# Huangying-Zhan/DF-VO

Measured on NVIDIA H100. Metric: VO frames/sec on 376x1241 pairs, higher is better.
Workload: dtype bf16 tensor-core convs (fp32 accumulate) + fp32 flow/selection + fp64 pose solvers

## Files before the change

df-vo_b200/csrc/conv_chain.cu:

```cuda
#include "tc_ptx.cuh"

#ifndef DFVO_HOSTSIM
#include <cuda.h>
#include <stdio.h>
#include <stdlib.h>
#include <string.h>

#include <vector>

namespace dfvo {

#define CHAIN_MAXL 12
#define CHAIN_THREADS 384
#define CHAIN_TH 16

struct ChainL {
  int N, H, W, tiles_x, tiles_y, n_blocks, ntiles;
  int nsrc, srcC[3];
  int kh, kw, dy0, dx0, HW, HH;
  int block_n;
  int Cout, Cout_pad, act, out_f32, zero_pad_to;
  const float* bias;
  void* out; long long oN, oH, oW;
  const void* res; long long rN, rH, rW;
// ... 97 lines not shown
      const int ntaps = p.kh * p.kw;
      const uint32_t b_bytes = (uint32_t)p.block_n * 128u;
      for (int tile = blockIdx.x; tile < p.ntiles; tile += gridDim.x) {
        const int nb = tile / (p.tiles_x * p.tiles_y * p.N);
        int kofs = 0;
        for (int s = 0; s < p.nsrc; ++s) {
          for (int c0 = 0; c0 < p.srcC[s]; c0 += 64) {
            for (int tap = 0; tap < ntaps; ++tap) {
              mbar_wait(rb.empty(), rb.ph ^ 1u);
              if (elect_one()) {
                mbar_expect_tx(rb.full(), b_bytes);
                tma_load_3d(rb.slot(), &P.tmB[l], rb.full(), kofs + c0, nb * p.block_n, tap);
              }
              __syncwarp();
              rb.next();
            }
          }
          kofs += p.srcC[s];
        }
      }
    }
  } else if (warp >= 4) {
    const int ct = threadIdx.x - 128, wg = ct >> 7, wq = (ct >> 5) & 3;
    const bool leader = (ct & 127) == 0;
    for (int l = 0; l < P.nlayers; ++l) {
      const ChainL& p = P.L[l];
      asm volatile("bar.sync 1, 256;" ::: "memory");
      for (int i = ct; i < p.Cout_pad; i += 256) bias_s[i] = p.bias ? p.bias[i] : 0.f;
      asm volatile("bar.sync 1, 256;" ::: "memory");
      if (l > 0 && p.res != nullptr) {
        if (lane == 0 && !chain_wait(P.bar + (l - 1), gridDim.x)) *P.err = 1u;
        __syncwarp();
      }
      TcEpi ep; ep.Cout = p.Cout; ep.zero_pad_to = p.zero_pad_to; ep.act = p.act; ep.out_f32 = p.out_f32; ep.round_tf32 = 0; ep.out = p.out; ep.res = p.res;
      switch (p.block_n) {
        case 16: chain_layer<S, 16>(p, ra, rb, ep, bias_s, wg, wq, lane, leader); break;
        case 32: chain_layer<S, 32>(p, ra, rb, ep, bias_s, wg, wq, lane, leader); break;
        case 64: chain_layer<S, 64>(p, ra, rb, ep, bias_s, wg, wq, lane, leader); break;
        case 128: if (S <= 2) chain_layer<S, (S <= 2 ? 128 : 16)>(p, ra, rb, ep, bias_s, wg, wq, lane, leader); break;
        default: if (S == 1) chain_layer<S, (S == 1 ? 256 : 16)>(p, ra, rb, ep, bias_s, wg, wq, lane, leader); break;
      }
      if (l + 1 < P.nlayers) {
        asm volatile("fence.proxy.async;" ::: "memory");
        __threadfence();
        asm volatile("bar.sync 1, 256;" ::: "memory");
        if (ct == 0) chain_arrive(P.bar + l);
      }
    }
  }
}

static int chain_env(const char* name, int dflt) {
  const char* v = getenv(name);
  return v ? atoi(v) : dflt;
}

static bool chain_rect(const ConvTc& c, int* kh, int* kw, int* dy0, int* dx0) {
  int ymin = 127, ymax = -128, xmin = 127, xmax = -128;
  for (int t = 0; t < c.ntaps; ++t) {
    if (c.dy[t] < ymin) ymin = c.dy[t];
    if (c.dy[t] > ymax) ymax = c.dy[t];
    if (c.dx[t] < xmin) xmin = c.dx[t];
    if (c.dx[t] > xmax) xmax = c.dx[t];
  }
  const int h = ymax - ymin + 1, w = xmax - xmin + 1;
  if (h * w != c.ntaps) return false;
  for (int t = 0; t < c.ntaps; ++t)
// ... 198 lines not shown
```

df-vo_b200/csrc/conv_halo.cu:

```cuda
#include "tc_ptx.cuh"

#ifndef DFVO_HOSTSIM
#include <cuda.h>
#include <stdio.h>
#include <stdlib.h>
#include <string.h>

namespace dfvo {

struct ConvHaloK {
  int N, H, W, tiles_x, tiles_y, n_blocks, ntiles;
  int nsrc, srcC[3];
  int kh, kw, dy0, dx0;
  int HW, HH;
  int a_stages, b_stages, a_stage_bytes;
  int Cout, Cout_pad, act, out_f32, zero_pad_to;
  int chunk;
  int esize, round_tf32;
  const float* bias;
  void* out; long long oN, oH, oW;
  const void* res; long long rN, rH, rW;
};

#define HALO_THREADS 384
#define HALO_TH 16

template <int S, int BN, int TF32, int MINB>
__global__ void __launch_bounds__(HALO_THREADS, MINB)
k_conv_halo(const __grid_constant__ CUtensorMap tmA0, const __grid_constant__ CUtensorMap tmA1,
            const __grid_constant__ CUtensorMap tmA2, const __grid_constant__ CUtensorMap tmB,
            const __grid_constant__ ConvHaloK p) {
  using namespace tc;
  extern __shared__ uint8_t smem_raw[];
  const uint32_t raw = smem_u32(smem_raw);
  const uint32_t base = (raw + 1023u) & ~1023u;
  uint8_t* base_ptr = smem_raw + (base - raw);
  const uint32_t b_stage_bytes = (uint32_t)BN * 128u;
  const uint32_t a_base = base;
  const uint32_t b_base = base + (uint32_t)p.a_stages * (uint32_t)p.a_stage_bytes;
  const uint32_t bar_base = b_base + (uint32_t)p.b_stages * b_stage_bytes;
  TcRing ra{a_base, (uint32_t)p.a_stage_bytes, bar_base, bar_base + 8u * (uint32_t)p.a_stages, p.a_stages, 0, 0u};
  TcRing rb{b_base, b_stage_bytes, bar_base + 16u * (uint32_t)p.a_stages, bar_base + 16u * (uint32_t)p.a_stages + 8u * (uint32_t)p.b_stages,
            p.b_stages, 0, 0u};
  float* bias_s = reinterpret_cast<float*>(base_ptr + (bar_base - base) + 16u * (uint32_t)(p.a_stages + p.b_stages));

  const int warp = threadIdx.x >> 5, lane = threadIdx.x & 31;

  pdl_trigger();

  if (warp == 0 && lane == 0) {
    prefetch_tmap(&tmA0); prefetch_tmap(&tmB);
// ... 20 lines not shown
          if (elect_one()) {
            mbar_expect_tx(ra.full(), a_bytes);
            tma_load_4d(ra.slot(), tm, ra.full(), c0, x0, y0, n);
          }
          __syncwarp();
          ra.next();
        }
      }
    }
  } else if (warp == 1) {
    for (int tile = blockIdx.x; tile < p.ntiles; tile += gridDim.x) {
      const int nb = tile / (p.tiles_x * p.tiles_y * p.N);
      int kofs = 0;
      for (int s = 0; s < p.nsrc; ++s) {
        for (int c0 = 0; c0 < p.srcC[s]; c0 += p.chunk) {
          for (int tap = 0; tap < ntaps; ++tap) {
            mbar_wait(rb.empty(), rb.ph ^ 1u);
            if (elect_one()) {
              mbar_expect_tx(rb.full(), b_stage_bytes);
              tma_load_3d(rb.slot(), &tmB, rb.full(), kofs + c0, nb * BN, tap);
            }
            __syncwarp();
            rb.next();
          }
        }
        kofs += p.srcC[s];
      }
    }
  } else if (warp >= 4) {
    const int ct = threadIdx.x - 128, wg = ct >> 7;
    for (int i = ct; i < p.Cout_pad; i += 256) bias_s[i] = p.bias ? p.bias[i] : 0.f;
    asm volatile("bar.sync 1, 256;" ::: "memory");
    TcEpi ep; ep.Cout = p.Cout; ep.zero_pad_to = p.zero_pad_to; ep.act = p.act; ep.out_f32 = p.out_f32; ep.round_tf32 = p.round_tf32; ep.out = p.out; ep.res = p.res;
    float acc[S][BN / 2];
    for (int tile = blockIdx.x; tile < p.ntiles; tile += gridDim.x) {
      halo_tile_mma<S, BN, TF32>(acc, ra, rb, p.nsrc, p.srcC, p.chunk, p.esize, p.kh, p.kw, p.HW, wg, (ct & 127) == 0);
      int t = tile;
      const int tx = t % p.tiles_x; t /= p.tiles_x;
      const int ty = t % p.tiles_y; t /= p.tiles_y;
      const int n = t % p.N; const int nb = t / p.N;
      halo_tile_store<S, BN>(acc, ep, bias_s, nb * BN, n, tx * 8 * S, ty * HALO_TH, p.W, p.H, p.oN, p.oH, p.oW, p.rN, p.rH, p.rW, wg,
                             (ct >> 5) & 3, lane);
    }
  }
}

static int env_int(const char* name, int dflt) {
  const char* v = getenv(name);
  return v ? atoi(v) : dflt;
}

static bool rect_taps(const ConvTc& c, int* kh, int* kw, int* dy0, int* dx0) {
  int ymin = 127, ymax = -128, xmin = 127, xmax = -128;
  for (int t = 0; t < c.ntaps; ++t) {
    if (c.dy[t] < ymin) ymin = c.dy[t];
    if (c.dy[t] > ymax) ymax = c.dy[t];
    if (c.dx[t] < xmin) xmin = c.dx[t];
    if (c.dx[t] > xmax) xmax = c.dx[t];
  }
  const int h = ymax - ymin + 1, w = xmax - xmin + 1;
  if (h * w != c.ntaps) return false;
  for (int t = 0; t < c.ntaps; ++t)
    if (c.dy[t] != ymin + t / w || c.dx[t] != xmin + t % w) return false;
  *kh = h; *kw = w; *dy0 = ymin; *dx0 = xmin;
  return true;
}

struct HaloCfg { int S, block_n, ctas, a_stages, b_stages, a_stage_bytes; size_t smem; double cost; };

static bool halo_fit(int S, int bn, int ctas, int kh, int kw, int Cout_pad, HaloCfg* out) {
  const int HW = 8 * S + kw - 1, HH = HALO_TH + kh - 1;
  if (HW > 256 || HH > 256) return false;
  const int a_stage = (HW * HH * 128 + 1023) & ~1023;
  const int b_stage = bn * 128;
  const size_t fixed = 1024 + 8 * 64 + (size_t)Cout_pad * 4;
// ... 78 lines not shown
#undef DFVO_HALO_CASE
  DFVO_REQUIRE(false, DFVO_EINVAL, "conv_halo: no kernel for S %d block_n %d with %d CTAs per SM", S, bn, ctas);
}

int conv_halo(const ConvTc& c, cudaStream_t s) {
  DFVO_REQUIRE(c.nsrc >= 1 && c.nsrc <= 3 && c.ntaps >= 1 && c.ntaps <= 49, DFVO_EINVAL, "conv_halo: nsrc/ntaps");
  DFVO_REQUIRE(c.Cout_pad % 16 == 0 && c.Cout_pad >= 16, DFVO_EINVAL, "conv_halo: Cout_pad %d must be a multiple of 16", c.Cout_pad);
  ConvHaloK k;
  memset(&k, 0, sizeof(k));
  DFVO_REQUIRE(rect_taps(c, &k.kh, &k.kw, &k.dy0, &k.dx0), DFVO_EINVAL, "conv_halo: taps are not a rectangle");
  HaloCfg h;
  DFVO_REQUIRE(halo_choose(c, k.kh, k.kw, &h), DFVO_EINVAL, "conv_halo: no tile configuration fits");
  const int S = h.S, bn = h.block_n;
  k.N = c.N; k.H = c.H; k.W = c.W;
  k.tiles_x = cdiv(c.W, 8 * S); k.tiles_y = cdiv(c.H, HALO_TH);
  k.n_blocks = c.Cout_pad / bn;
  k.ntiles = k.tiles_x * k.tiles_y * c.N * k.n_blocks;
  k.HW = 8 * S + k.kw - 1; k.HH = HALO_TH + k.kh - 1;
  k.a_stages = h.a_stages; k.b_stages = h.b_stages; k.a_stage_bytes = h.a_stage_bytes;
  k.nsrc = c.nsrc;
  const int es = c.esize == 4 ? 4 : 2;
  k.esize = es; k.chunk = 128 / es; k.round_tf32 = c.round_out_tf32;
  int ktot = 0;
  for (int i = 0; i < c.nsrc; ++i) {
    DFVO_REQUIRE(c.src[i].C % 16 == 0 && c.src[i].C > 0, DFVO_EINVAL, "conv_halo: source %d channels %d not a multiple of 16", i, c.src[i].C);
    DFVO_REQUIRE(((uintptr_t)c.src[i].p & 15) == 0 && (c.src[i].sW * es) % 16 == 0 && (c.src[i].sH * es) % 16 == 0 && (c.src[i].sN * es) % 16 == 0,
                 DFVO_EINVAL, "conv_halo: source %d not 16-byte aligned/strided", i);
    k.srcC[i] = c.src[i].C; ktot += c.src[i].C;
  }
  k.Cout = c.Cout; k.Cout_pad = c.Cout_pad; k.act = c.act; k.out_f32 = c.out_f32;
  k.zero_pad_to = c.zero_pad_to > c.Cout ? c.zero_pad_to : c.Cout;
  k.bias = c.bias; k.out = c.out; k.oN = c.oN; k.oH = c.oH; k.oW = c.oW;
  k.res = c.residual; k.rN = c.rN; k.rH = c.rH; k.rW = c.rW;

  CUtensorMap tmA[3], tmB;
  for (int i = 0; i < 3; ++i) {
    const ConvTcSource& src = c.src[i < c.nsrc ? i : 0];
    const int inW = c.inW > 0 ? c.inW : c.W, inH = c.inH > 0 ? c.inH : c.H;
    unsigned long long dims[4] = {(unsigned long long)src.C, (unsigned long long)inW, (unsigned long long)inH, (unsigned long long)c.N};
    unsigned long long str[3] = {(unsigned long long)src.sW * es, (unsigned long long)src.sH * es, (unsigned long long)src.sN * es};
    unsigned box[4] = {(unsigned)k.chunk, (unsigned)k.HW, (unsigned)k.HH, 1};
    int rc = tc_encode_map(&tmA[i], src.p, 4, dims, str, box, es);
    if (rc) return rc;
  }
  {
    unsigned long long dims[3] = {(unsigned long long)ktot, (unsigned long long)c.Cout_pad, (unsigned long long)c.ntaps};
    unsigned long long str[2] = {(unsigned long long)ktot * es, (unsigned long long)ktot * es * (unsigned long long)c.Cout_pad};
    unsigned box[3] = {(unsigned)k.chunk, (unsigned)bn, 1};
    int rc = tc_encode_map(&tmB, c.w, 3, dims, str, box, es);
    if (rc) return rc;
  }
  const int slots = h.ctas * tc_num_sms();
  const int grid = k.ntiles < slots ? k.ntiles : slots;
  ++g_launch_count;
  TcProf pr;
  const bool prof = tc_prof_begin(s, &pr);
  const int rc = es == 4 ? launch_halo_t<1>(S, bn, h.ctas, tmA, tmB, k, grid, h.smem, s) : launch_halo_t<0>(S, bn, h.ctas, tmA, tmB, k, grid, h.smem, s);
  if (rc) return rc;
  if (prof) {
    char d[256];
    snprintf(d, sizeof(d), "halo%s N%d %dx%d k%dx%d src[%d,%d,%d] cout%d/%d bn%d S%d stages%d/%d grid%d tiles%d ctas%d gflop %.3f", es == 4 ? "-tf32" : "", c.N, c.H, c.W,
             k.kh, k.kw, c.src[0].C, c.nsrc > 1 ? c.src[1].C : 0, c.nsrc > 2 ? c.src[2].C : 0, c.Cout, c.Cout_pad, bn,
             S, k.a_stages, k.b_stages, grid, k.ntiles, h.ctas, c.flops * 1e-9);
    tc_prof_end(s, pr, c.flops, d);
  }
  DFVO_CHECK_LAUNCH();
  return DFVO_OK;
}

}
#endif
```

df-vo_b200/csrc/conv_tc.cu:

```cuda
#include "tc_ptx.cuh"

#ifndef DFVO_HOSTSIM
#include <cuda.h>
#endif
#include <stdio.h>
#include <stdlib.h>
#include <string.h>

#include <string>
#include <utility>
#include <vector>

namespace dfvo {

void conv_tc_tile_shape(int H, int W, int* tw, int* th) {
  long long best = -1;
  int bw = 128, bh = 1;
  for (int w = 128; w >= 1; w >>= 1) {
    int h = 128 / w;
    long long area = (long long)cdiv(W, w) * w * (long long)cdiv(H, h) * h;
    if (best < 0 || area < best) { best = area; bw = w; bh = h; }
  }
  *tw = bw; *th = bh;
}

struct ConvTcK {
  int N, H, W, tw, th, tiles_x, tiles_y, n_blocks, ntiles;
  int nsrc, srcC[3];
  int ntaps;
  int8_t dy[49], dx[49];
  int8_t py[49], px[49];
  int stride, src_pitch;
  int block_n, stages;
  int Cout, Cout_pad, act, out_f32, zero_pad_to;
  int chunk, esize, round_tf32;
  const float* bias;
  void* out; long long oN, oH, oW;
  const void* res; long long rN, rH, rW;
};

#ifndef DFVO_HOSTSIM
#define TC_THREADS 384
#define TC_A_BYTES 16384

template <int BN, int TF32, int NKS>
__device__ __forceinline__ void tc_stage_mma(float (&acc)[1][BN / 2], uint32_t at, uint32_t bt, uint32_t fresh) {
  using namespace tc;
  wgmma_fence();
  halo_tap_mma<1, BN, TF32, NKS>(acc, at, bt, 1024u, fresh);
  wgmma_commit();
  wgmma_wait<1>();
}

template <int BN, int TF32>
__global__ void __launch_bounds__(TC_THREADS, 1)
k_conv_tc(const __grid_constant__ CUtensorMap tmA0, const __grid_constant__ CUtensorMap tmA1,
          const __grid_constant__ CUtensorMap tmA2, const __grid_constant__ CUtensorMap tmB,
          const __grid_constant__ ConvTcK p) {
  using namespace tc;
  extern __shared__ uint8_t smem_raw[];
  const uint32_t raw = smem_u32(smem_raw);
  const uint32_t base = (raw + 1023u) & ~1023u;
  uint8_t* base_ptr = smem_raw + (base - raw);
  const uint32_t stage_bytes = TC_A_BYTES + (uint32_t)BN * 128u;
  const uint32_t bar_base = base + (uint32_t)p.stages * stage_bytes;
  auto full_bar = [&](int s) { return bar_base + 8u * (uint32_t)s; };
  auto empty_bar = [&](int s) { return bar_base + 8u * (uint32_t)(p.stages + s); };
  float* bias_s = reinterpret_cast<float*>(base_ptr + (size_t)p.stages * stage_bytes + 8u * (2 * p.stages) + 64);
// ... 16 lines not shown
      int t = tile;
      const int tx = t % p.tiles_x; t /= p.tiles_x;
      const int ty = t % p.tiles_y; t /= p.tiles_y;
      const int n = t % p.N; const int nb = t / p.N;
      const int x0 = tx * p.tw, y0 = ty * p.th;
      for (int tap = 0; tap < p.ntaps; ++tap) {
        int kofs = 0;
        for (int s = 0; s < p.nsrc; ++s) {
          const CUtensorMap* tm = s == 0 ? &tmA0 : (s == 1 ? &tmA1 : &tmA2);
          for (int c0 = 0; c0 < p.srcC[s]; c0 += p.chunk) {
            mbar_wait(empty_bar(stage), phase ^ 1u);
            if (elect_one()) {
              const uint32_t sa = base + (uint32_t)stage * stage_bytes;
              mbar_expect_tx(full_bar(stage), stage_bytes);
              if (p.stride == 2)
                tma_load_5d(sa, tm, full_bar(stage), c0 + p.px[tap] * p.src_pitch, x0 + p.dx[tap], p.py[tap], y0 + p.dy[tap], n);
              else
                tma_load_4d(sa, tm, full_bar(stage), c0, x0 + p.dx[tap], y0 + p.dy[tap], n);
              tma_load_3d(sa + TC_A_BYTES, &tmB, full_bar(stage), kofs + c0, nb * BN, tap);
            }
            __syncwarp();
            if (++stage == p.stages) { stage = 0; phase ^= 1u; }
          }
          kofs += p.srcC[s];
        }
      }
    }
  } else if (warp >= 4) {
    const int ct = threadIdx.x - 128, wg = ct >> 7, wq = (ct >> 5) & 3;
    const bool leader = (ct & 127) == 0;
    for (int i = ct; i < p.Cout_pad; i += 256) bias_s[i] = p.bias ? p.bias[i] : 0.f;
    asm volatile("bar.sync 1, 256;" ::: "memory");
    TcEpi ep; ep.Cout = p.Cout; ep.zero_pad_to = p.zero_pad_to; ep.act = p.act; ep.out_f32 = p.out_f32; ep.round_tf32 = p.round_tf32; ep.out = p.out; ep.res = p.res;
    int stage = 0; uint32_t phase = 0;
    float acc[BN / 2];
    for (int tile = blockIdx.x; tile < p.ntiles; tile += gridDim.x) {
      uint32_t fresh = 0;
      int pend = -1;
      for (int tap = 0; tap < p.ntaps; ++tap) {
        for (int s = 0; s < p.nsrc; ++s) {
          for (int c0 = 0; c0 < p.srcC[s]; c0 += p.chunk) {
            mbar_wait(full_bar(stage), phase);
            const uint32_t sa = base + (uint32_t)stage * stage_bytes;
            const int rem = p.srcC[s] - c0;
            const int nks = ((rem >= p.chunk ? p.chunk : rem) * p.esize) >> 5;
            float (&acc1)[1][BN / 2] = reinterpret_cast<float (&)[1][BN / 2]>(acc);
            const uint32_t at = sa + (uint32_t)wg * 8192u, bt = sa + TC_A_BYTES;
            switch (nks) {
              case 4: tc_stage_mma<BN, TF32, 4>(acc1, at, bt, fresh); break;
              case 3: tc_stage_mma<BN, TF32, 3>(acc1, at, bt, fresh); break;
              case 2: tc_stage_mma<BN, TF32, 2>(acc1, at, bt, fresh); break;
              default: tc_stage_mma<BN, TF32, 1>(acc1, at, bt, fresh); break;
            }
            if (pend >= 0 && leader) mbar_arrive(empty_bar(pend));
            pend = stage;
            fresh = 1u;
            if (++stage == p.stages) { stage = 0; phase ^= 1u; }
          }
        }
      }
      wgmma_wait<0>();
      if (leader) mbar_arrive(empty_bar(pend));

      int t = tile;
      const int tx = t % p.tiles_x; t /= p.tiles_x;
      const int ty = t % p.tiles_y; t /= p.tiles_y;
      const int n = t % p.N; const int nb = t / p.N;
#pragma unroll
      for (int h = 0; h < 2; ++h) {
        const int row = 64 * wg + 16 * wq + (lane >> 2) + 8 * h;
        const int x = tx * p.tw + (row % p.tw), y = ty * p.th + (row / p.tw);
        if (x >= p.W || y >= p.H) continue;
        const long long opix = n * p.oN + y * p.oH + x * p.oW, rpix = n * p.rN + y * p.rH + x * p.rW;
#pragma unroll
        for (int j = 0; j < BN / 8; ++j)
          tc_store2(ep, bias_s, acc[4 * j + 2 * h], acc[4 * j + 2 * h + 1], nb * BN + 8 * j + 2 * (lane & 3), opix, rpix);
      }
    }
  }
}

typedef CUresult (*PFN_encodeTiled)(CUtensorMap*, CUtensorMapDataType, cuuint32_t, void*, const cuuint64_t*,
                                    const cuuint64_t*, const cuuint32_t*, const cuuint32_t*, CUtensorMapInterleave,
                                    CUtensorMapSwizzle, CUtensorMapL2promotion, CUtensorMapFloatOOBfill);

static PFN_encodeTiled get_encode() {
  static PFN_encodeTiled fn = nullptr;
  if (!fn) {
    void* p = nullptr;
    cudaDriverEntryPointQueryResult qres;
    if (cudaGetDriverEntryPoint("cuTensorMapEncodeTiled", &p, cudaEnableDefault, &qres) == cudaSuccess &&
        qres == cudaDriverEntryPointSuccess)
      fn = (PFN_encodeTiled)p;
  }
  return fn;
}

int tc_encode_map(void* map, const void* ptr, int rank, const unsigned long long* dims_, const unsigned long long* strides_, const unsigned* box_,
                  int esize, int swizzle_bytes) {
  cuuint64_t dims[5], str[5];
  cuuint32_t box[5];
  for (int i = 0; i < rank; ++i) { dims[i] = dims_[i]; box[i] = box_[i]; if (i < rank - 1) str[i] = strides_[i]; }
  CUtensorMap* m = reinterpret_cast<CUtensorMap*>(map);
  const cuuint64_t* strides_bytes = str;
  PFN_encodeTiled enc = get_encode();
  DFVO_REQUIRE(enc != nullptr, DFVO_ECUDA, "cuTensorMapEncodeTiled entry point unavailable");
  cuuint32_t es[5] = {1, 1, 1, 1, 1};
  CUresult r = enc(m, esize == 4 ? CU_TENSOR_MAP_DATA_TYPE_FLOAT32 : CU_TENSOR_MAP_DATA_TYPE_BFLOAT16, (cuuint32_t)rank, const_cast<void*>(ptr), dims, strides_bytes, box, es,
                   CU_TENSOR_MAP_INTERLEAVE_NONE,
                   swizzle_bytes == 32 ? CU_TENSOR_MAP_SWIZZLE_32B : (swizzle_bytes == 64 ? CU_TENSOR_MAP_SWIZZLE_64B : CU_TENSOR_MAP_SWIZZLE_128B),
                   CU_TENSOR_MAP_L2_PROMOTION_L2_256B,
                   CU_TENSOR_MAP_FLOAT_OOB_FILL_NONE);
  DFVO_REQUIRE(r == CUDA_SUCCESS, DFVO_ECUDA, "cuTensorMapEncodeTiled failed: %d (rank %d dims %llu %llu %llu box %u %u %u)", (int)r,
               rank, (unsigned long long)dims[0], (unsigned long long)dims[1], (unsigned long long)dims[2], box[0], box[1], box[2]);
  return DFVO_OK;
}

struct ConvTcPlanImpl {
  CUtensorMap tmA[3], tmB;
  ConvTcK k;
  int grid;
  size_t smem;
};

static int g_num_sms = 0;
void tc_launch_config(cudaLaunchConfig_t* cfg, cudaLaunchAttribute* attr, int grid, int block, size_t smem, cudaStream_t s) {
  static int pdl = -1;
  if (pdl < 0) { const char* e = getenv("DFVO_PDL"); pdl = !(e && atoi(e) == 0); }
  memset(cfg, 0, sizeof(*cfg));
  cfg->gridDim = dim3(grid); cfg->blockDim = dim3(block); cfg->dynamicSmemBytes = smem; cfg->stream = s;
  attr->id = cudaLaunchAttributeProgrammaticStreamSerialization;
  attr->val.programmaticStreamSerializationAllowed = 1;
  cfg->attrs = attr; cfg->numAttrs = pdl ? 1 : 0;
}
int tc_num_sms() {
  if (!g_num_sms) {
    int dev = 0; cudaGetDevice(&dev);
    cudaDeviceGetAttribute(&g_num_sms, cudaDevAttrMultiProcessorCount, dev);
    if (g_num_sms <= 0) g_num_sms = 132;
  }
  return g_num_sms;
}
static int encode_map(CUtensorMap* m, const void* ptr, int rank, const cuuint64_t* dims, const cuuint64_t* strides_bytes, const cuuint32_t* box,
                      int esize) {
  unsigned long long d[5], st[5]; unsigned b[5];
  for (int i = 0; i < rank; ++i) { d[i] = dims[i]; b[i] = box[i]; if (i < rank - 1) st[i] = strides_bytes[i]; }
  return tc_encode_map(m, ptr, rank, d, st, b, esize, 128);
}

static int build_plan(const ConvTc& c, ConvTcPlanImpl* pl) {
  DFVO_REQUIRE(c.nsrc >= 1 && c.nsrc <= 3 && c.ntaps >= 1 && c.ntaps <= 49, DFVO_EINVAL, "conv_tc: nsrc/ntaps");
  DFVO_REQUIRE(c.Cout_pad % 16 == 0 && c.Cout_pad >= 16, DFVO_EINVAL, "conv_tc: Cout_pad %d must be a multiple of 16", c.Cout_pad);
  ConvTcK& k = pl->k;
  memset(&k, 0, sizeof(k));
  k.N = c.N; k.H = c.H; k.W = c.W;
  conv_tc_tile_shape(c.H, c.W, &k.tw, &k.th);
  k.tiles_x = cdiv(c.W, k.tw); k.tiles_y = cdiv(c.H, k.th);
  k.block_n = 256;
  while (c.Cout_pad % k.block_n) k.block_n >>= 1;
  k.n_blocks = c.Cout_pad / k.block_n;
  k.ntiles = k.tiles_x * k.tiles_y * c.N * k.n_blocks;
  k.nsrc = c.nsrc; k.ntaps = c.ntaps;
  const int es = c.esize == 4 ? 4 : 2;
  k.esize = es; k.chunk = 128 / es; k.round_tf32 = c.round_out_tf32;
  int ktot = 0;
  for (int s = 0; s < c.nsrc; ++s) {
    DFVO_REQUIRE(c.src[s].C % 16 == 0 && c.src[s].C > 0, DFVO_EINVAL, "conv_tc: source %d channels %d not a multiple of 16", s, c.src[s].C);
    DFVO_REQUIRE(((uintptr_t)c.src[s].p & 15) == 0 && (c.src[s].sW * es) % 16 == 0 && (c.src[s].sH * es) % 16 == 0 && (c.src[s].sN * es) % 16 == 0,
                 DFVO_EINVAL, "conv_tc: source %d not 16-byte aligned/strided", s);
    k.srcC[s] = c.src[s].C; ktot += c.src[s].C;
  }
  k.stride = c.stride == 2 ? 2 : 1;
  if (k.stride == 2) {
    const int inH = c.inH > 0 ? c.inH : 2 * c.H, inW = c.inW > 0 ? c.inW : 2 * c.W;
    DFVO_REQUIRE(c.nsrc == 1 && inH % 2 == 0 && inW % 2 == 0 && inH == 2 * c.H && inW == 2 * c.W, DFVO_EINVAL,
                 "conv_tc stride 2: needs one source and even input size = 2x output");
    DFVO_REQUIRE(c.src[0].sH == (long long)inW * c.src[0].sW, DFVO_EINVAL, "conv_tc stride 2: rows must be contiguous");
    k.src_pitch = (int)c.src[0].sW;
    for (int t = 0; t < c.ntaps; ++t) {
      const int oy = c.dy[t], ox = c.dx[t];
      k.py[t] = (int8_t)(((oy % 2) + 2) % 2); k.dy[t] = (int8_t)((oy - k.py[t]) / 2);
      k.px[t] = (int8_t)(((ox % 2) + 2) % 2); k.dx[t] = (int8_t)((ox - k.px[t]) / 2);
    }
  } else {
    memcpy(k.dy, c.dy, sizeof(k.dy)); memcpy(k.dx, c.dx, sizeof(k.dx));
  }
  k.Cout = c.Cout; k.Cout_pad = c.Cout_pad; k.act = c.act; k.out_f32 = c.out_f32;
  k.zero_pad_to = c.zero_pad_to > c.Cout ? c.zero_pad_to : c.Cout;
  k.bias = c.bias; k.out = c.out; k.oN = c.oN; k.oH = c.oH; k.oW = c.oW;
  k.res = c.residual; k.rN = c.rN; k.rH = c.rH; k.rW = c.rW;
  const size_t stage_bytes = TC_A_BYTES + (size_t)k.block_n * 128;
  const size_t fixed = 1024  + 8 * 64  + 64 + (size_t)c.Cout_pad * 4 ;
  int stages = (int)((200 * 1024 - fixed) / stage_bytes);
  if (stages > 8) stages = 8;
  DFVO_REQUIRE(stages >= 2, DFVO_EINVAL, "conv_tc: tile does not fit in shared memory");
  k.stages = stages;
  pl->smem = fixed + (size_t)stages * stage_bytes;
  pl->grid = k.ntiles < tc_num_sms() ? k.ntiles : tc_num_sms();
  for (int s = 0; s < 3; ++s) {
    const ConvTcSource& src = c.src[s < c.nsrc ? s : 0];
    if (k.stride == 2) {
      const int inW2 = c.W, inH2 = c.H;
      cuuint64_t dims[5] = {(cuuint64_t)(src.sW + src.C), (cuuint64_t)inW2, 2, (cuuint64_t)inH2, (cuuint64_t)c.N};
      cuuint64_t str[4] = {(cuuint64_t)src.sW * 2 * es, (cuuint64_t)src.sH * es, (cuuint64_t)src.sH * 2 * es, (cuuint64_t)src.sN * es};
      cuuint32_t box[5] = {(cuuint32_t)k.chunk, (cuuint32_t)k.tw, 1, (cuuint32_t)k.th, 1};
      int rc = encode_map(&pl->tmA[s], src.p, 5, dims, str, box, es);
      if (rc) return rc;
      continue;
    }
    const int inW = c.inW > 0 ? c.inW : c.W, inH = c.inH > 0 ? c.inH : c.H;
    cuuint64_t dims[4] = {(cuuint64_t)src.C, (cuuint64_t)inW, (cuuint64_t)inH, (cuuint64_t)c.N};
    cuuint64_t str[3] = {(cuuint64_t)src.sW * es, (cuuint64_t)src.sH * es, (cuuint64_t)src.sN * es};
    cuuint32_t box[4] = {(cuuint32_t)k.chunk, (cuuint32_t)k.tw, (cuuint32_t)k.th, 1};
    int rc = encode_map(&pl->tmA[s], src.p, 4, dims, str, box, es);
    if (rc) return rc;
  }
  {
    cuuint64_t dims[3] = {(cuuint64_t)ktot, (cuuint64_t)c.Cout_pad, (cuuint64_t)c.ntaps};
    cuuint64_t str[2] = {(cuuint64_t)ktot * es, (cuuint64_t)ktot * es * (cuuint64_t)c.Cout_pad};
    cuuint32_t box[3] = {(cuuint32_t)k.chunk, (cuuint32_t)k.block_n, 1};
    int rc = encode_map(&pl->tmB, c.w, 3, dims, str, box, es);
    if (rc) return rc;
  }
// ... 144 lines not shown
```

df-vo_b200/csrc/tc_ptx.cuh:

```cuda
#pragma once
#include "ops.h"
#ifndef DFVO_HOSTSIM
#include "wgmma.cuh"
#endif

namespace dfvo {

struct TcEpi {
  int Cout, zero_pad_to, act, out_f32;
  int round_tf32;
  void* out;
  const void* res;
};

#ifndef DFVO_HOSTSIM
namespace tc {

__device__ __forceinline__ uint32_t smem_u32(const void* p) { return (uint32_t)__cvta_generic_to_shared(p); }

__device__ __forceinline__ void mbar_init(uint32_t bar, uint32_t count) {
  asm volatile("mbarrier.init.shared::cta.b64 [%0], %1;" ::"r"(bar), "r"(count));
}
__device__ __forceinline__ void mbar_expect_tx(uint32_t bar, uint32_t bytes) {
  asm volatile("mbarrier.arrive.expect_tx.shared::cta.b64 _, [%0], %1;" ::"r"(bar), "r"(bytes) : "memory");
}
__device__ __forceinline__ void mbar_arrive(uint32_t bar) {
  asm volatile("mbarrier.arrive.shared::cta.b64 _, [%0];" ::"r"(bar) : "memory");
}
__device__ __forceinline__ void mbar_wait(uint32_t bar, uint32_t parity) {
  asm volatile(
      "{\n\t.reg .pred p;\n\t"
      "WAIT_%=:\n\t"
      "mbarrier.try_wait.parity.shared::cta.b64 p, [%0], %1;\n\t"
      "@p bra DONE_%=;\n\t"
      "bra WAIT_%=;\n\t"
      "DONE_%=:\n\t}" ::"r"(bar), "r"(parity) : "memory");
}
__device__ __forceinline__ void tma_load_4d(uint32_t dst, const void* tmap, uint32_t bar, int c0, int c1, int c2, int c3) {
  asm volatile(
      "cp.async.bulk.tensor.4d.shared::cluster.global.mbarrier::complete_tx::bytes [%0], [%1, {%3, %4, %5, %6}], [%2];"
      ::"r"(dst), "l"((uint64_t)tmap), "r"(bar), "r"(c0), "r"(c1), "r"(c2), "r"(c3) : "memory");
}
__device__ __forceinline__ void tma_load_5d(uint32_t dst, const void* tmap, uint32_t bar, int c0, int c1, int c2, int c3, int c4) {
// ... 41 lines not shown
  const bool two = c + 1 < p.zero_pad_to;
  float v[2] = {a, b};
#pragma unroll
  for (int j = 0; j < 2; ++j) {
    if (c + j < p.Cout) {
      float x = v[j] + bias[c + j];
      if (p.res) x += p.out_f32 ? reinterpret_cast<const float*>(p.res)[rpix + c + j]
                                : __bfloat162float(reinterpret_cast<const __nv_bfloat16*>(p.res)[rpix + c + j]);
      v[j] = apply_act(x, p.act);
    } else {
      v[j] = 0.f;
    }
  }
  if (p.out_f32) {
    if (p.round_tf32) { v[0] = tc::tc_round_tf32(v[0]); v[1] = tc::tc_round_tf32(v[1]); }
    float* o = reinterpret_cast<float*>(p.out) + opix + c;
    if (two && (reinterpret_cast<uintptr_t>(o) & 7u) == 0) {
      *reinterpret_cast<float2*>(o) = make_float2(v[0], v[1]);
    } else {
      o[0] = v[0];
      if (two) o[1] = v[1];
    }
  } else {
    __nv_bfloat16* o = reinterpret_cast<__nv_bfloat16*>(p.out) + opix + c;
    if (two && (reinterpret_cast<uintptr_t>(o) & 3u) == 0) {
      *reinterpret_cast<__nv_bfloat162*>(o) = __floats2bfloat162_rn(v[0], v[1]);
    } else {
      o[0] = __float2bfloat16_rn(v[0]);
      if (two) o[1] = __float2bfloat16_rn(v[1]);
    }
  }
}

struct TcRing {
  uint32_t base, slot_bytes, full0, empty0;
  int n, i;
  uint32_t ph;
  __device__ __forceinline__ uint32_t slot() const { return base + (uint32_t)i * slot_bytes; }
  __device__ __forceinline__ uint32_t full() const { return full0 + 8u * (uint32_t)i; }
  __device__ __forceinline__ uint32_t empty() const { return empty0 + 8u * (uint32_t)i; }
  __device__ __forceinline__ void next() { if (++i == n) { i = 0; ph ^= 1u; } }
};

template <int S, int BN, int TF32, int NKS>
__device__ __forceinline__ void halo_tap_mma(float (&acc)[S][BN / 2], uint32_t at, uint32_t bt, uint32_t a_sbo, uint32_t fresh) {
  using namespace tc;
#pragma unroll
  for (int sub = 0; sub < S; ++sub)
#pragma unroll
    for (int ks = 0; ks < NKS; ++ks)
      Wgmma<BN, TF32>::mma(acc[sub], desc_sw128(at + (uint32_t)sub * 1024u + 32u * ks, a_sbo), desc_sw128(bt + 32u * ks, 1024u),
                           ks == 0 ? fresh : 1u);
}

template <int S, int BN, int TF32, int NKS>
__device__ __forceinline__ void halo_chunk_mma(float (&acc)[S][BN / 2], TcRing& rb, uint32_t a0, uint32_t a_sbo, int kh, int kw, int HW,
                                               uint32_t& fresh, bool leader) {
  using namespace tc;
  int pend = -1;
  for (int ky = 0; ky < kh; ++ky) {
    for (int kx = 0; kx < kw; ++kx) {
      mbar_wait(rb.full(), rb.ph);
      wgmma_fence();
      halo_tap_mma<S, BN, TF32, NKS>(acc, a0 + (uint32_t)(ky * HW + kx) * 128u, rb.slot(), a_sbo, fresh);
      wgmma_commit();
      wgmma_wait<1>();
      if (pend >= 0 && leader) mbar_arrive(rb.empty0 + 8u * (uint32_t)pend);
      pend = rb.i;
      rb.next();
      fresh = 1u;
    }
  }
  wgmma_wait<0>();
  if (leader) mbar_arrive(rb.empty0 + 8u * (uint32_t)pend);
}

template <int S, int BN, int TF32>
__device__ __forceinline__ void halo_tile_mma(float (&acc)[S][BN / 2], TcRing& ra, TcRing& rb, int nsrc, const int* srcC, int chunk,
                                              int esize, int kh, int kw, int HW, int wg, bool leader) {
  using namespace tc;
  const uint32_t a_sbo = (uint32_t)HW * 128u;
  uint32_t fresh = 0;
  for (int s = 0; s < nsrc; ++s) {
    for (int c0 = 0; c0 < srcC[s]; c0 += chunk) {
      const int rem = srcC[s] - c0;
      const int nks = ((rem >= chunk ? chunk : rem) * esize) >> 5;
      mbar_wait(ra.full(), ra.ph);
      const uint32_t a0 = ra.slot() + (uint32_t)wg * 8u * a_sbo;
      switch (nks) {
        case 4: halo_chunk_mma<S, BN, TF32, 4>(acc, rb, a0, a_sbo, kh, kw, HW, fresh, leader); break;
        case 3: halo_chunk_mma<S, BN, TF32, 3>(acc, rb, a0, a_sbo, kh, kw, HW, fresh, leader); break;
        case 2: halo_chunk_mma<S, BN, TF32, 2>(acc, rb, a0, a_sbo, kh, kw, HW, fresh, leader); break;
        default: halo_chunk_mma<S, BN, TF32, 1>(acc, rb, a0, a_sbo, kh, kw, HW, fresh, leader); break;
      }
      if (leader) mbar_arrive(ra.empty());
      ra.next();
    }
  }
}

template <int S, int BN>
__device__ __forceinline__ void halo_tile_store(const float (&acc)[S][BN / 2], const TcEpi& ep, const float* bias_s, int cbase, int n,
                                                int x0, int y0, int W, int H, long long oN, long long oH, long long oW, long long rN,
                                                long long rH, long long rW, int wg, int warp_in_wg, int lane) {
#pragma unroll
  for (int h = 0; h < 2; ++h) {
    const int y = y0 + 8 * wg + 2 * warp_in_wg + h;
    if (y >= H) continue;
#pragma unroll
    for (int sub = 0; sub < S; ++sub) {
      const int x = x0 + 8 * sub + (lane >> 2);
      if (x >= W) continue;
      const long long opix = n * oN + y * oH + x * oW, rpix = n * rN + y * rH + x * rW;
#pragma unroll
      for (int j = 0; j < BN / 8; ++j)
        tc_store2(ep, bias_s, acc[sub][4 * j + 2 * h], acc[sub][4 * j + 2 * h + 1], cbase + 8 * j + 2 * (lane & 3), opix, rpix);
    }
  }
}

#endif

int conv_halo(const ConvTc& c, cudaStream_t s);
bool conv_halo_supported(const ConvTc& c);
struct TcProf { cudaEvent_t e0, e1; };
bool tc_prof_begin(cudaStream_t s, TcProf* p);
void tc_prof_end(cudaStream_t s, const TcProf& p, double flops, const char* desc);
int tc_encode_map(void* map, const void* ptr, int rank, const unsigned long long* dims, const unsigned long long* strides_bytes,
                  const unsigned* box, int esize = 2, int swizzle_bytes = 128);
int tc_num_sms();
#ifndef DFVO_HOSTSIM
void tc_launch_config(cudaLaunchConfig_t* cfg, cudaLaunchAttribute* attr, int grid, int block, size_t smem, cudaStream_t s);
#endif

}
```

Measured before the change: 229.6.

## Vectorize conv epilogue stores via quad shuffles and defer halo ring releases

Adds a 16-byte vectorized epilogue path. Quad-lane shuffles transpose wgmma accumulator fragments so each thread writes 8 contiguous channels, with vectorized residual loads, whenever outputs and residuals are aligned and the tile is full. The halo kernel's MMA loop no longer drains with wgmma_wait<0> after every chunk. B-slot and A-slot releases are deferred across chunk boundaries, so tensor-core work stays in flight between input chunks. Optional clock64 stamping instrumentation is compiled in behind a macro. The cost is extra shuffle instructions and more complex barrier bookkeeping.

Result: faster. 279.1 (median of 6 runs) (+21.6%).

```diff
diff --git a/df-vo_b200/csrc/conv_chain.cu b/df-vo_b200/csrc/conv_chain.cu
--- a/df-vo_b200/csrc/conv_chain.cu
+++ b/df-vo_b200/csrc/conv_chain.cu
@@ -153,7 +153,7 @@
         if (lane == 0 && !chain_wait(P.bar + (l - 1), gridDim.x)) *P.err = 1u;
         __syncwarp();
       }
-      TcEpi ep; ep.Cout = p.Cout; ep.zero_pad_to = p.zero_pad_to; ep.act = p.act; ep.out_f32 = p.out_f32; ep.round_tf32 = 0; ep.out = p.out; ep.res = p.res;
+      TcEpi ep; ep.Cout = p.Cout; ep.zero_pad_to = p.zero_pad_to; ep.act = p.act; ep.out_f32 = p.out_f32; ep.round_tf32 = 0; ep.vec16 = 0; ep.out = p.out; ep.res = p.res;
       switch (p.block_n) {
         case 16: chain_layer<S, 16>(p, ra, rb, ep, bias_s, wg, wq, lane, leader); break;
         case 32: chain_layer<S, 32>(p, ra, rb, ep, bias_s, wg, wq, lane, leader); break;
diff --git a/df-vo_b200/csrc/conv_halo.cu b/df-vo_b200/csrc/conv_halo.cu
--- a/df-vo_b200/csrc/conv_halo.cu
+++ b/df-vo_b200/csrc/conv_halo.cu
@@ -17,6 +17,7 @@
   int Cout, Cout_pad, act, out_f32, zero_pad_to;
   int chunk;
   int esize, round_tf32;
+  int vec16;
   const float* bias;
   void* out; long long oN, oH, oW;
   const void* res; long long rN, rH, rW;
@@ -103,8 +104,10 @@
     for (int i = ct; i < p.Cout_pad; i += 256) bias_s[i] = p.bias ? p.bias[i] : 0.f;
     asm volatile("bar.sync 1, 256;" ::: "memory");
     TcEpi ep; ep.Cout = p.Cout; ep.zero_pad_to = p.zero_pad_to; ep.act = p.act; ep.out_f32 = p.out_f32; ep.round_tf32 = p.round_tf32; ep.out = p.out; ep.res = p.res;
+    ep.vec16 = p.vec16;
     float acc[S][BN / 2];
-    for (int tile = blockIdx.x; tile < p.ntiles; tile += gridDim.x) {
+    for (int tile = blockIdx.x, it = 0; tile < p.ntiles; tile += gridDim.x, ++it) {
+      DFVO_HALO_STAMP(0);
       halo_tile_mma<S, BN, TF32>(acc, ra, rb, p.nsrc, p.srcC, p.chunk, p.esize, p.kh, p.kw, p.HW, wg, (ct & 127) == 0);
       int t = tile;
       const int tx = t % p.tiles_x; t /= p.tiles_x;
@@ -112,6 +115,8 @@
       const int n = t % p.N; const int nb = t / p.N;
       halo_tile_store<S, BN>(acc, ep, bias_s, nb * BN, n, tx * 8 * S, ty * HALO_TH, p.W, p.H, p.oN, p.oH, p.oW, p.rN, p.rH, p.rW, wg,
                              (ct >> 5) & 3, lane);
+      DFVO_HALO_STAMP(5);
+      DFVO_HALO_STAMP_TILE(it);
     }
   }
 }
@@ -256,6 +261,7 @@
   k.zero_pad_to = c.zero_pad_to > c.Cout ? c.zero_pad_to : c.Cout;
   k.bias = c.bias; k.out = c.out; k.oN = c.oN; k.oH = c.oH; k.oW = c.oW;
   k.res = c.residual; k.rN = c.rN; k.rH = c.rH; k.rW = c.rW;
+  k.vec16 = tc_epi_vec16(c);
 
   CUtensorMap tmA[3], tmB;
   for (int i = 0; i < 3; ++i) {
@@ -293,4 +299,16 @@
 }
 
 }
+
+#ifdef DFVO_HALO_STAMPS
+extern "C" int dfvo_halo_stamps_read(unsigned long long* host, int* dims) {
+  dims[0] = HALO_STAMP_CTAS; dims[1] = HALO_STAMP_TILES; dims[2] = HALO_STAMP_N;
+  if (!host) return 0;
+  if (cudaDeviceSynchronize() != cudaSuccess) return 1;
+  if (cudaMemcpyFromSymbol(host, dfvo::tc::g_halo_stamps, sizeof(dfvo::tc::g_halo_stamps)) != cudaSuccess) return 1;
+  void* dev = nullptr;
+  if (cudaGetSymbolAddress(&dev, dfvo::tc::g_halo_stamps) != cudaSuccess) return 1;
+  return cudaMemset(dev, 0, sizeof(dfvo::tc::g_halo_stamps)) == cudaSuccess ? 0 : 1;
+}
 #endif
+#endif
diff --git a/df-vo_b200/csrc/conv_tc.cu b/df-vo_b200/csrc/conv_tc.cu
--- a/df-vo_b200/csrc/conv_tc.cu
+++ b/df-vo_b200/csrc/conv_tc.cu
@@ -34,6 +34,7 @@
   int block_n, stages;
   int Cout, Cout_pad, act, out_f32, zero_pad_to;
   int chunk, esize, round_tf32;
+  int vec16;
   const float* bias;
   void* out; long long oN, oH, oW;
   const void* res; long long rN, rH, rW;
@@ -116,6 +117,7 @@
     for (int i = ct; i < p.Cout_pad; i += 256) bias_s[i] = p.bias ? p.bias[i] : 0.f;
     asm volatile("bar.sync 1, 256;" ::: "memory");
     TcEpi ep; ep.Cout = p.Cout; ep.zero_pad_to = p.zero_pad_to; ep.act = p.act; ep.out_f32 = p.out_f32; ep.round_tf32 = p.round_tf32; ep.out = p.out; ep.res = p.res;
+    ep.vec16 = p.vec16;
     int stage = 0; uint32_t phase = 0;
     float acc[BN / 2];
     for (int tile = blockIdx.x; tile < p.ntiles; tile += gridDim.x) {
@@ -150,6 +152,15 @@
       const int tx = t % p.tiles_x; t /= p.tiles_x;
       const int ty = t % p.tiles_y; t /= p.tiles_y;
       const int n = t % p.N; const int nb = t / p.N;
+      if (ep.vec16 && (nb + 1) * BN <= p.Cout && (tx + 1) * p.tw <= p.W && (ty + 1) * p.th <= p.H) {
+        float (&acc1)[1][BN / 2] = reinterpret_cast<float (&)[1][BN / 2]>(acc);
+        tc_store_frag16<BN>(ep, bias_s, acc1[0], nb * BN, lane, [&](int h, long long* opix, long long* rpix) {
+          const int row = 64 * wg + 16 * wq + (lane >> 2) + 8 * h;
+          const int x = tx * p.tw + (row % p.tw), y = ty * p.th + (row / p.tw);
+          *opix = n * p.oN + y * p.oH + x * p.oW; *rpix = n * p.rN + y * p.rH + x * p.rW;
+        });
+        continue;
+      }
 #pragma unroll
       for (int h = 0; h < 2; ++h) {
         const int row = 64 * wg + 16 * wq + (lane >> 2) + 8 * h;
@@ -216,6 +227,13 @@
   attr->id = cudaLaunchAttributeProgrammaticStreamSerialization;
   attr->val.programmaticStreamSerializationAllowed = 1;
   cfg->attrs = attr; cfg->numAttrs = pdl ? 1 : 0;
+}
+bool tc_epi_vec16(const ConvTc& c) {
+  const long long es = c.out_f32 ? 4 : 2;
+  auto aligned = [&](const void* p, long long sN, long long sH, long long sW) {
+    return ((uintptr_t)p & 15) == 0 && (sN * es) % 16 == 0 && (sH * es) % 16 == 0 && (sW * es) % 16 == 0;
+  };
+  return aligned(c.out, c.oN, c.oH, c.oW) && (!c.residual || aligned(c.residual, c.rN, c.rH, c.rW));
 }
 int tc_num_sms() {
   if (!g_num_sms) {
@@ -273,6 +291,7 @@
   k.zero_pad_to = c.zero_pad_to > c.Cout ? c.zero_pad_to : c.Cout;
   k.bias = c.bias; k.out = c.out; k.oN = c.oN; k.oH = c.oH; k.oW = c.oW;
   k.res = c.residual; k.rN = c.rN; k.rH = c.rH; k.rW = c.rW;
+  k.vec16 = tc_epi_vec16(c);
   const size_t stage_bytes = TC_A_BYTES + (size_t)k.block_n * 128;
   const size_t fixed = 1024  + 8 * 64  + 64 + (size_t)c.Cout_pad * 4 ;
   int stages = (int)((200 * 1024 - fixed) / stage_bytes);
diff --git a/df-vo_b200/csrc/tc_ptx.cuh b/df-vo_b200/csrc/tc_ptx.cuh
--- a/df-vo_b200/csrc/tc_ptx.cuh
+++ b/df-vo_b200/csrc/tc_ptx.cuh
@@ -9,6 +9,7 @@
 struct TcEpi {
   int Cout, zero_pad_to, act, out_f32;
   int round_tf32;
+  int vec16;
   void* out;
   const void* res;
 };
@@ -116,6 +117,91 @@
   }
 }
 
+__device__ __forceinline__ void tc_quad_transpose(float (&v)[8], int q) {
+#pragma unroll
+  for (int b = 0; b < 2; ++b) {
+    const bool bq = (q >> b) & 1;
+#pragma unroll
+    for (int lo = 0; lo < 4; ++lo) {
+      if (lo & (1 << b)) continue;
+      const int hi = lo | (1 << b);
+#pragma unroll
+      for (int e = 0; e < 2; ++e) {
+        const float r = __shfl_xor_sync(0xffffffffu, bq ? v[2 * lo + e] : v[2 * hi + e], 1 << b);
+        if (bq) v[2 * lo + e] = r; else v[2 * hi + e] = r;
+      }
+    }
+  }
+}
+
+template <int ACT>
+__device__ __forceinline__ void tc_store8(const TcEpi& p, const float* bias, float (&v)[8], int c, long long opix, long long rpix) {
+  uint4 rb16 = make_uint4(0u, 0u, 0u, 0u);
+  if (p.res && !p.out_f32) rb16 = *reinterpret_cast<const uint4*>(reinterpret_cast<const __nv_bfloat16*>(p.res) + rpix + c);
+#pragma unroll
+  for (int k = 0; k < 2; ++k) {
+    float r[4];
+    if (p.res) {
+      if (p.out_f32) {
+        const float4 r4 = reinterpret_cast<const float4*>(reinterpret_cast<const float*>(p.res) + rpix + c)[k];
+        r[0] = r4.x; r[1] = r4.y; r[2] = r4.z; r[3] = r4.w;
+      } else {
+        const uint32_t w0 = k ? rb16.z : rb16.x, w1 = k ? rb16.w : rb16.y;
+        const __nv_bfloat162 b0 = *reinterpret_cast<const __nv_bfloat162*>(&w0), b1 = *reinterpret_cast<const __nv_bfloat162*>(&w1);
+        r[0] = __low2float(b0); r[1] = __high2float(b0); r[2] = __low2float(b1); r[3] = __high2float(b1);
+      }
+    }
+#pragma unroll
+    for (int e = 0; e < 4; ++e) {
+      float x = v[4 * k + e] + bias[c + 4 * k + e];
+      if (p.res) x += r[e];
+      v[4 * k + e] = apply_act(x, ACT);
+    }
+  }
+  if (p.out_f32) {
+    if (p.round_tf32) {
+#pragma unroll
+      for (int e = 0; e < 8; ++e) v[e] = tc::tc_round_tf32(v[e]);
+    }
+    float4* o = reinterpret_cast<float4*>(reinterpret_cast<float*>(p.out) + opix + c);
+    o[0] = make_float4(v[0], v[1], v[2], v[3]);
+    o[1] = make_float4(v[4], v[5], v[6], v[7]);
+  } else {
+    uint32_t w[4];
+#pragma unroll
+    for (int k = 0; k < 4; ++k) {
+      const __nv_bfloat162 b2 = __floats2bfloat162_rn(v[2 * k], v[2 * k + 1]);
+      w[k] = *reinterpret_cast<const uint32_t*>(&b2);
+    }
+    *reinterpret_cast<uint4*>(reinterpret_cast<__nv_bfloat16*>(p.out) + opix + c) = make_uint4(w[0], w[1], w[2], w[3]);
+  }
+}
+
+template <int BN, int ACT, typename Pix>
+__device__ __forceinline__ void tc_store_frag16_act(const TcEpi& p, const float* bias, const float (&acc)[BN / 2], int cbase, int lane,
+                                                    Pix pix) {
+  const int q = lane & 3, h = q & 1;
+  long long opix, rpix;
+  pix(h, &opix, &rpix);
+#pragma unroll
+  for (int g = 0; g < BN / 16; ++g) {
+    float v[8];
+#pragma unroll
+    for (int k = 0; k < 8; ++k) v[k] = acc[8 * g + k];
+    tc_quad_transpose(v, q);
+    tc_store8<ACT>(p, bias, v, cbase + 8 * (2 * g + (q >> 1)), opix, rpix);
+  }
+}
+template <int BN, typename Pix>
+__device__ __forceinline__ void tc_store_frag16(const TcEpi& p, const float* bias, const float (&acc)[BN / 2], int cbase, int lane, Pix pix) {
+  switch (p.act) {
+    case ACT_LEAKY: tc_store_frag16_act<BN, ACT_LEAKY>(p, bias, acc, cbase, lane, pix); break;
+    case ACT_RELU: tc_store_frag16_act<BN, ACT_RELU>(p, bias, acc, cbase, lane, pix); break;
+    case ACT_ELU: tc_store_frag16_act<BN, ACT_ELU>(p, bias, acc, cbase, lane, pix); break;
+    case ACT_SIGMOID: tc_store_frag16_act<BN, ACT_SIGMOID>(p, bias, acc, cbase, lane, pix); break;
+    default: tc_store_frag16_act<BN, ACT_NONE>(p, bias, acc, cbase, lane, pix); break;
+  }
+}
 struct TcRing {
   uint32_t base, slot_bytes, full0, empty0;
   int n, i;
@@ -126,6 +212,39 @@
   __device__ __forceinline__ void next() { if (++i == n) { i = 0; ph ^= 1u; } }
 };
 
+#ifdef DFVO_HALO_STAMPS
+#define HALO_STAMP_CTAS 288
+#define HALO_STAMP_TILES 128
+#define HALO_STAMP_N 6
+namespace tc {
+static __device__ unsigned long long g_halo_stamps[HALO_STAMP_CTAS][2][HALO_STAMP_TILES + 1][HALO_STAMP_N];
+__device__ __forceinline__ unsigned long long* halo_stamp_row(int row) {
+  return g_halo_stamps[blockIdx.x % HALO_STAMP_CTAS][(threadIdx.x >> 7) & 1][row];
+}
+}
+#define DFVO_HALO_STAMP(k) \
+  do { if ((threadIdx.x & 127) == 0) tc::halo_stamp_row(HALO_STAMP_TILES)[k] = clock64(); } while (0)
+#define DFVO_HALO_TIMED(k, stmt)                                                                                  \
+  do {                                                                                                            \
+    const long long t0_ = clock64();                                                                              \
+    stmt;                                                                                                         \
+    if ((threadIdx.x & 127) == 0) tc::halo_stamp_row(HALO_STAMP_TILES)[k] += clock64() - t0_;                     \
+  } while (0)
+#define DFVO_HALO_STAMP_TILE(it)                                                                                  \
+  do {                                                                                                            \
+    if ((threadIdx.x & 127) == 0) {                                                                               \
+      unsigned long long* cur_ = tc::halo_stamp_row(HALO_STAMP_TILES);                                            \
+      if ((it) < HALO_STAMP_TILES)                                                                                \
+        for (int k_ = 0; k_ < HALO_STAMP_N; ++k_) tc::halo_stamp_row(it)[k_] = cur_[k_];                          \
+      cur_[2] = cur_[3] = 0;                                                                                      \
+    }                                                                                                             \
+  } while (0)
+#else
+#define DFVO_HALO_STAMP(k) do {} while (0)
+#define DFVO_HALO_TIMED(k, stmt) do { stmt; } while (0)
+#define DFVO_HALO_STAMP_TILE(it) do {} while (0)
+#endif
+
 template <int S, int BN, int TF32, int NKS>
 __device__ __forceinline__ void halo_tap_mma(float (&acc)[S][BN / 2], uint32_t at, uint32_t bt, uint32_t a_sbo, uint32_t fresh) {
   using namespace tc;
@@ -138,25 +257,26 @@
 }
 
 template <int S, int BN, int TF32, int NKS>
-__device__ __forceinline__ void halo_chunk_mma(float (&acc)[S][BN / 2], TcRing& rb, uint32_t a0, uint32_t a_sbo, int kh, int kw, int HW,
-                                               uint32_t& fresh, bool leader) {
+__device__ __forceinline__ void halo_chunk_mma(float (&acc)[S][BN / 2], const TcRing& ra, TcRing& rb, uint32_t a0, uint32_t a_sbo, int kh,
+                                               int kw, int HW, uint32_t& fresh, uint32_t& pend_b, bool leader) {
   using namespace tc;
-  int pend = -1;
+  const bool prev_a = fresh != 0u;
   for (int ky = 0; ky < kh; ++ky) {
     for (int kx = 0; kx < kw; ++kx) {
-      mbar_wait(rb.full(), rb.ph);
+      DFVO_HALO_TIMED(3, mbar_wait(rb.full(), rb.ph));
       wgmma_fence();
       halo_tap_mma<S, BN, TF32, NKS>(acc, a0 + (uint32_t)(ky * HW + kx) * 128u, rb.slot(), a_sbo, fresh);
       wgmma_commit();
       wgmma_wait<1>();
-      if (pend >= 0 && leader) mbar_arrive(rb.empty0 + 8u * (uint32_t)pend);
-      pend = rb.i;
+      if (leader) {
+        if (pend_b) mbar_arrive(pend_b);
+        if (prev_a && ky == 0 && kx == 0) mbar_arrive(ra.empty0 + 8u * (uint32_t)(ra.i ? ra.i - 1 : ra.n - 1));
+      }
+      pend_b = rb.empty();
       rb.next();
       fresh = 1u;
     }
   }
-  wgmma_wait<0>();
-  if (leader) mbar_arrive(rb.empty0 + 8u * (uint32_t)pend);
 }
 
 template <int S, int BN, int TF32>
@@ -165,21 +285,28 @@
   using namespace tc;
   const uint32_t a_sbo = (uint32_t)HW * 128u;
   uint32_t fresh = 0;
+  uint32_t pend_b = 0u;
   for (int s = 0; s < nsrc; ++s) {
     for (int c0 = 0; c0 < srcC[s]; c0 += chunk) {
       const int rem = srcC[s] - c0;
       const int nks = ((rem >= chunk ? chunk : rem) * esize) >> 5;
-      mbar_wait(ra.full(), ra.ph);
+      DFVO_HALO_TIMED(2, mbar_wait(ra.full(), ra.ph));
+      if (s == 0 && c0 == 0) DFVO_HALO_STAMP(1);
       const uint32_t a0 = ra.slot() + (uint32_t)wg * 8u * a_sbo;
       switch (nks) {
-        case 4: halo_chunk_mma<S, BN, TF32, 4>(acc, rb, a0, a_sbo, kh, kw, HW, fresh, leader); break;
-        case 3: halo_chunk_mma<S, BN, TF32, 3>(acc, rb, a0, a_sbo, kh, kw, HW, fresh, leader); break;
-        case 2: halo_chunk_mma<S, BN, TF32, 2>(acc, rb, a0, a_sbo, kh, kw, HW, fresh, leader); break;
-        default: halo_chunk_mma<S, BN, TF32, 1>(acc, rb, a0, a_sbo, kh, kw, HW, fresh, leader); break;
+        case 4: halo_chunk_mma<S, BN, TF32, 4>(acc, ra, rb, a0, a_sbo, kh, kw, HW, fresh, pend_b, leader); break;
+        case 3: halo_chunk_mma<S, BN, TF32, 3>(acc, ra, rb, a0, a_sbo, kh, kw, HW, fresh, pend_b, leader); break;
+        case 2: halo_chunk_mma<S, BN, TF32, 2>(acc, ra, rb, a0, a_sbo, kh, kw, HW, fresh, pend_b, leader); break;
+        default: halo_chunk_mma<S, BN, TF32, 1>(acc, ra, rb, a0, a_sbo, kh, kw, HW, fresh, pend_b, leader); break;
       }
-      if (leader) mbar_arrive(ra.empty());
       ra.next();
     }
+  }
+  wgmma_wait<0>();
+  DFVO_HALO_STAMP(4);
+  if (leader) {
+    mbar_arrive(pend_b);
+    mbar_arrive(ra.empty0 + 8u * (uint32_t)(ra.i ? ra.i - 1 : ra.n - 1));
   }
 }
 
@@ -187,14 +314,21 @@
 __device__ __forceinline__ void halo_tile_store(const float (&acc)[S][BN / 2], const TcEpi& ep, const float* bias_s, int cbase, int n,
                                                 int x0, int y0, int W, int H, long long oN, long long oH, long long oW, long long rN,
                                                 long long rH, long long rW, int wg, int warp_in_wg, int lane) {
-#pragma unroll
-  for (int h = 0; h < 2; ++h) {
-    const int y = y0 + 8 * wg + 2 * warp_in_wg + h;
-    if (y >= H) continue;
-#pragma unroll
-    for (int sub = 0; sub < S; ++sub) {
-      const int x = x0 + 8 * sub + (lane >> 2);
-      if (x >= W) continue;
+  const int yw = y0 + 8 * wg + 2 * warp_in_wg;
+  const bool vec = ep.vec16 && cbase + BN <= ep.Cout && yw + 1 < H;
+#pragma unroll
+  for (int sub = 0; sub < S; ++sub) {
+    const int x = x0 + 8 * sub + (lane >> 2);
+    if (vec && x0 + 8 * sub + 8 <= W) {
+      tc_store_frag16<BN>(ep, bias_s, acc[sub], cbase, lane, [&](int h, long long* opix, long long* rpix) {
+        *opix = n * oN + (yw + h) * oH + x * oW; *rpix = n * rN + (yw + h) * rH + x * rW;
+      });
+      continue;
+    }
+#pragma unroll
+    for (int h = 0; h < 2; ++h) {
+      const int y = yw + h;
+      if (y >= H || x >= W) continue;
       const long long opix = n * oN + y * oH + x * oW, rpix = n * rN + y * rH + x * rW;
 #pragma unroll
       for (int j = 0; j < BN / 8; ++j)
@@ -213,6 +347,7 @@
 int tc_encode_map(void* map, const void* ptr, int rank, const unsigned long long* dims, const unsigned long long* strides_bytes,
                   const unsigned* box, int esize = 2, int swizzle_bytes = 128);
 int tc_num_sms();
+bool tc_epi_vec16(const ConvTc& c);
 #ifndef DFVO_HOSTSIM
 void tc_launch_config(cudaLaunchConfig_t* cfg, cudaLaunchAttribute* attr, int grid, int block, size_t smem, cudaStream_t s);
 #endif
```
